# paullric/tempestmodel

Measured on AMD Instinct MI355X. Metric: element-DOF-updates/s (JW baroclinic wave ne30 np4 L30, ARS343 IMEX), higher is better.
Workload: dtype f64

## Files before the change

include/tempest_mi355x.h:

```cpp
#ifndef TEMPEST_MI355X_H
#define TEMPEST_MI355X_H

#ifdef __cplusplus
extern "C" {
#endif

#define TMX_ABI_VERSION 5

#define TMX_OK                 0
#define TMX_ERR_INVALID       -1
#define TMX_ERR_UNSUPPORTED   -2
#define TMX_ERR_DEVICE        -3
#define TMX_ERR_SINGULAR      -4
#define TMX_ERR_COMM          -5

typedef struct tmx_engine tmx_engine;

enum {
	TMX_OP_INTERP_NODE_TO_REDGE = 0,
	TMX_OP_INTERP_REDGE_TO_NODE,
	TMX_OP_DIFF_NODE_TO_NODE,
	TMX_OP_DIFF_NODE_TO_REDGE,
	TMX_OP_DIFF_REDGE_TO_NODE,
	TMX_OP_DIFF_REDGE_TO_REDGE,
// ... 181 lines not shown
	TMX_INFO_COLUMN_KERNEL,
	TMX_INFO_COLUMN_VARIANT
};
long long tmx_info(tmx_engine * e, int what);

int tmx_set_option(tmx_engine * e, const char * name, double value);
int tmx_get_option(tmx_engine * e, const char * name, double * value);
typedef void (*tmx_dgbsv_fn)(const int * n, const int * kl, const int * ku, const int * nrhs, double * ab, const int * ldab, int * ipiv,
	double * b, const int * ldb, int * info);
int tmx_lu_flavour_from_dgbsv(tmx_engine * e, tmx_dgbsv_fn dgbsv);
int tmx_options_report(tmx_engine * e, char * buf, int cap);
int tmx_options_from_environment(tmx_engine * e);

int tmx_plan_get(tmx_engine * e, int what, int * out, int cap);
int tmx_plan_get_matrices(tmx_engine * e, double * out, int cap);
int tmx_debug_unique_tables(tmx_engine * e, int tile_shape, int what, int * out, int cap);
int tmx_debug_program_unique(int scheme, int first_step, int last_step);
int tmx_debug_program_mixed(int scheme, int first_step, int last_step, int instance);
int tmx_debug_program_rayleigh(int scheme, int first_step, int last_step);
int tmx_debug_program_prefix(int scheme, int first_step, int last_step, int * pairs, int * terms, int cap);
int tmx_debug_h_timing(tmx_engine * e, unsigned long long * out);
int tmx_debug_h_walk_timing(tmx_engine * e, unsigned long long * out);

int tmx_debug_dss_loopback(tmx_engine ** engines, int n, int instance);
int tmx_debug_loopback_group(tmx_engine ** engines, int n);
int tmx_debug_comm_selftest(tmx_engine * e);

int tmx_debug_pivot_stats(tmx_engine * e, int enable, unsigned long long out[2]);

int tmx_debug_program_copies(int scheme, int mode, int steps, int share, int * copies, int * shared);
int tmx_debug_dcmip_node_coefficients(int panel, double alpha, double beta, double * out);
int tmx_debug_dcmip_tsurf(double lat, double * out);

enum {
	TMX_K_H_EXPLICIT = 0, TMX_K_V_EXPLICIT, TMX_K_VI_ASSEMBLE, TMX_K_VI_SOLVE, TMX_K_DSS,
	TMX_K_HYPERVIS, TMX_K_LINCOMB, TMX_K_EXCHANGE, TMX_K_COUNT
};
int tmx_profile_enable(tmx_engine * e, int on);
int tmx_profile_get(tmx_engine * e, int kernel, double * total_ms, long long * launches);
int tmx_profile_reset(tmx_engine * e);

#ifdef __cplusplus
}
#endif
#endif
```

tempestmodel_amd/csrc/tmx_host.hip:

```cpp
#include "tmx_hostshared.h"


static thread_local std::string g_err;

void tmx_set_error(const char * fmt, ...) {
	char buf[1024];
	va_list ap;
	va_start(ap, fmt);
	vsnprintf(buf, sizeof(buf), fmt, ap);
	va_end(ap);
	g_err = buf;
}

extern "C" const char * tmx_last_error(void) { return g_err.c_str(); }




NcclApi g_nccl;

int load_rccl() {
	if (g_nccl.Send) return TMX_OK;
	void * h = dlopen(nullptr, RTLD_NOW | RTLD_GLOBAL);
	if (!h || !dlsym(h, "ncclSend")) {
// ... 884 lines not shown
			int n = 0;
			if (e->comm && g_nccl.CommCount && g_nccl.CommCount(e->comm, &n) == 0) return n;
			return 0;
		}
		case TMX_INFO_SEND_COLUMNS: return e->nsend;
		case TMX_INFO_HALO_TRANSPORT: return (e->cfg.n_ranks == 1) ? 0 : (e->lb ? 3 : (e->p2p ? 2 : (e->comm ? 1 : 0)));
	}
	return -1;
}

extern "C" int tmx_debug_h_timing(tmx_engine * e, unsigned long long * out) {
	int r; if ((r = check_ready(e))) return r;
	HIPCHK(hipStreamSynchronize(e->stream));
	tmxk_h_timing_read(out);
	return TMX_OK;
}
extern "C" int tmx_debug_h_walk_timing(tmx_engine * e, unsigned long long * out) {
	int r; if ((r = check_ready(e))) return r;
	HIPCHK(hipStreamSynchronize(e->stream));
	tmxk_h_walk_timing_read(out);
	return TMX_OK;
}

extern "C" int tmx_debug_pivot_stats(tmx_engine * e, int enable, unsigned long long out[2]) {
	int r; if ((r = check_ready(e))) return r;
	HIPCHK(hipStreamSynchronize(e->stream));
	if (out) {
		out[0] = out[1] = 0;
		if (e->d_pivot_stats) HIPCHK(hipMemcpy(out, e->d_pivot_stats, 2 * sizeof(unsigned long long), hipMemcpyDeviceToHost));
	}
#ifdef TMX_PAIR_TIMING
	const size_t stat_words = 2 + 8 * 4096;
	if (e->d_pivot_stats && !enable) {
		std::vector<unsigned long long> rec(stat_words);
		HIPCHK(hipMemcpy(rec.data(), e->d_pivot_stats, stat_words * sizeof(unsigned long long), hipMemcpyDeviceToHost));
		for (size_t w = 0; w < 4096; w++) {
			const unsigned long long * q = &rec[2 + 8 * w];
			if (q[0]) fprintf(stderr, "pairtiming wave %zu role %llu hw_id %llx xcc %llu work %llu wait %llu forward %llu back %llu\n", w, q[0] - 1, q[1], q[2], q[3], q[4], q[5], q[6]);
		}
		if (e->vi_split_back) {
			const int n = TMX_FTOT * (e->L + 1);
			for (int g : { 0, 100, 400 }) {
				std::vector<int> m(n);
				HIPCHK(hipMemcpy(m.data(), (const int *)e->d_rhs + (size_t)g * n, n * sizeof(int), hipMemcpyDeviceToHost));
				fprintf(stderr, "umask group %d:", g);
				for (int j = 0; j < n; j++) fprintf(stderr, " %x", m[j] >> 4);
// ... 34 lines not shown
```

tempestmodel_amd/csrc/tmx_internal.h:

```cpp
#pragma once
#include <hip/hip_runtime.h>
#include <string>
#include <vector>
#include "../../include/tempest_mi355x.h"

#define TMX_NP 4
#define TMX_NQ 16
#define TMX_TILE 64
#define TMX_FLAG_SINGULAR 1
#define TMX_FLAG_COMM 2
#define TMX_FTOT 3
#define TMX_BW 9

#define TMX_SLAB_U(L,k) (k)
#define TMX_SLAB_V(L,k) ((L) + (k))
#define TMX_SLAB_T(L,k) (2 * (L) + (k))
#define TMX_SLAB_R(L,k) (3 * (L) + (k))
#define TMX_SLAB_W(L,k) (4 * (L) + (k))
#define TMX_SLAB_Q(L,c,k) (5 * (L) + 1 + (c) * (L) + (k))

enum { G2_J2D = 0, G2_F, G2_C2A0, G2_C2A1, G2_C2B1, G2_JN, G2_JE, G2_DRX, G2_ZS,
	G2_LAT, G2_PS,
	G2_SINLAT, G2_COSLAT,
	G2_MP, G2_MA, G2_MB, G2_MC, G2_DAZ, G2_DBZ, G2_IDX, G2_IDX2,
// ... 58 lines not shown
	int b_ngroups = 0, b_ngroups_local = 0, nblocks = 0, nb_early = 0, nb_late = 0;
	int * d_b_sdst = nullptr, * d_b_sred = nullptr, * d_blk_info = nullptr, * d_b_gsrc = nullptr, * d_b_gdst = nullptr, * d_b_gn = nullptr, * d_b_gx = nullptr, * d_b_gtype = nullptr;
	int * d_blks_early = nullptr, * d_blks_late = nullptr;
	bool vite_ok = true;
	bool slots_by_blocks = false;
	int block_option = -1;
	size_t ustride = 0;
	double * d_ustate = nullptr, * d_part = nullptr, * d_g2d_t = nullptr, * d_g2d_u = nullptr;
	int * d_t_ucol = nullptr, * d_t_sdst = nullptr, * d_t_sred = nullptr;
	int * d_t_tinfo = nullptr;
	int * d_t_dcol = nullptr;
	int * d_ucol_of_dcol = nullptr;
	int * d_u_rep = nullptr;
	int * d_slot_ucol = nullptr;
	int * d_gsrc = nullptr, * d_gdst = nullptr, * d_gn = nullptr, * d_gx = nullptr, * d_gtype = nullptr;
	int * d_send_slots = nullptr;
	int * d_quads_early = nullptr, * d_quads_late = nullptr; int n_early = 0, n_late = 0; bool split = false;
	int * d_check = nullptr;
	std::vector<char> form;
	std::vector<int> uslot; int uspare = 0;
	int uprefix = 0, prefix_option = 1;
	long long prefix_for = -1;
	long long prefix_stages = 0;
	int n_uform = 0;
	long long conversions = 0;
	int backoff = 0, skip_steps = 0;
	unsigned dlive = 0u;
	int mixed_option = 1;
	long long mixed_steps = 0;
	bool physics_dirty = true, physics_ok = false;
	double * d_surf_u = nullptr;
};

struct PlanHost {
	std::vector<int> grp_cols, grp_n, grp_x, grp_type;
	std::vector<double> xmat;
	std::vector<int> send_nodes;
	std::vector<int> recv_nodes;
	std::vector<int> send_cols;
	std::vector<int> ucol, udep;
	std::vector<int> colref;
	std::vector<int> hvblocks;
	std::vector<int> quads_early, quads_late;
	std::vector<int> send_base, send_stride, ghost_base, ghost_stride;
};

// ... 155 lines not shown
#define TMX_EXP 1
#else
#define TMX_EXP 0
#endif
static inline bool tmxu_blocks_on(const tmx_engine * e, int which = 0) {
	if (!TMX_EXP || !e->u.built) return false;
	const int o = e->u.block_option;
	if (o == 2) return which != 2;
	if (o == 3) return which != 1;
	return o == 1 || (o < 0 && e->u.tile_shape == 4);
}

struct EmitTerms { double * xp; double coef[12]; int first; };
void tmxk_h_explicit(tmx_engine * e, const KParams & p, const double * xin, const double * xbase, double * xup, double dt, int fuse_v,
	int nterms = 0, const double * const * src = nullptr, const double * coef = nullptr, int premul = 0,
	const double * xin_uv = nullptr, const double * xbase_uv = nullptr, const double * const * src_uv = nullptr, const EmitTerms * emit = nullptr,
	unsigned dmask = 0u);
bool tmxk_h_walk_ok(const tmx_engine * e, const KParams & p, int fuse_v, int nterms, bool emit);
void tmxk_h_walk_prepare(tmx_engine * e, const KParams & p);
int tmxk_h_walk_segments(const tmx_engine * e, const KParams & p, int ntiles, int nterms, int waves_per_simd = 0);
void tmxk_h_walk(tmx_engine * e, const KParams & p, const double * xin, const double * xbase, double * xup, double dt, int fuse_v,
	int nterms, const double * const * src, const double * coef, int premul, const double * xin_uv, const double * xbase_uv, const double * const * src_uv, unsigned dmask,
	const EmitTerms * emit = nullptr);
bool tmxk_h_walk_fuses_udiff(const tmx_engine * e, const KParams & p, int fuse_v, int nterms);
bool tmxk_hv_walk_ok(const tmx_engine * e, const KParams & p);
void tmxk_hv_walk(tmx_engine * e, const KParams & p, const double * xsrc, const double * xbase, double * xout, double dt, double nu_s, double nu_d, double nu_v, int scale);
void tmxk_h_walk_timing_read(unsigned long long * out);
void tmxk_h_timing_read(unsigned long long * out);
void tmxk_sw_explicit(tmx_engine * e, const KParams & p, const double * xin, const double * xbase, double * xup, double dt);
void tmxk_v_explicit(tmx_engine * e, const KParams & p, const double * xin, double * xup, double dt, bool with_udiff_uv = false);
void tmxk_vi_assemble(tmx_engine * e, const KParams & p, const double * xin, double dt);
void tmxk_vi_solve(tmx_engine * e, const KParams & p, const double * xin, double * xup);
void tmxk_vi_fused(tmx_engine * e, const KParams & p, const double * xin, double * xup, double dt);
void tmxk_vi_terms_explicit(tmx_engine * e, const KParams & p, const double * xin, double * xup, double dt, bool with_uv = false);
void tmxk_dss(tmx_engine * e, const KParams & p, double * x, int g0, int g1);
void tmxk_hypervis(tmx_engine * e, const KParams & p, const double * xsrc, const double * xbase, double * xout,
	double dt, double nu_s, double nu_d, double nu_v, int scale_locally, bool pull_dss = false);
void tmxk_lincomb(tmx_engine * e, size_t n, double * dst, int nterms, const double * const * src, const double * coef, int dst_is_term0);
void tmxk_pack(tmx_engine * e, const KParams & p, const double * x);
void tmxk_pack_p2p(tmx_engine * e, const KParams & p, const double * x, int buf);
void tmxk_p2p_signal_wait(tmx_engine * e, hipStream_t s, int buf, unsigned long long seq);
void tmxk_rayleigh(tmx_engine * e, const KParams & p, double * x, double dt, const double * xs = nullptr, size_t NSS = 0, const int * ucd = nullptr);
void tmxk_held_suarez(tmx_engine * e, const KParams & p, double * x, const double * surf, double dt, const double * xs = nullptr, size_t NSS = 0, const int * ucd = nullptr);
void tmxk_kessler(tmx_engine * e, const KParams & p, double * x, double dt);
enum { DC_RA0 = 0, DC_RA1, DC_RB0, DC_RB1, DC_RCOS, DC_ADIV, DC_AA0, DC_AA1, DC_AB0, DC_AB1, DC_TSURF1, TMX_DC_NCOEF };
#define TMX_DC_NW 20
// ... 25 lines not shown
```

tempestmodel_amd/csrc/tmx_k_hwalk.hip:

```cpp
#include "tmx_device.h"

#ifdef TMX_H_TIMING
#define HW_WAVES 32768
__device__ unsigned long long g_hw_rec[8][HW_WAVES][8];
#define HW_DECL long long hw_ = __builtin_readcyclecounter(); long long hws_[7] = { 0, 0, 0, 0, 0, 0, 0 }
#define HW_MARK(i) do { const long long t1_ = __builtin_readcyclecounter(); hws_[i] += t1_ - hw_; hw_ = t1_; } while (0)
#define HW_END(NT_) do { if (threadIdx.x == 0) { const unsigned w_ = blockIdx.x % HW_WAVES; \
	for (int q_ = 0; q_ < 7; q_++) g_hw_rec[(NT_) & 7][w_][q_] = (unsigned long long)hws_[q_]; g_hw_rec[(NT_) & 7][w_][7] = 1ull; } } while (0)
void tmxk_h_walk_timing_read(unsigned long long * out) {
	static std::vector<unsigned long long> h((size_t)8 * HW_WAVES * 8);
	hipMemcpyFromSymbol(h.data(), HIP_SYMBOL(g_hw_rec), h.size() * sizeof(unsigned long long));
	for (int i = 0; i < 128; i++) out[i] = 0;
	for (int nt = 0; nt < 8; nt++) for (int w = 0; w < HW_WAVES; w++) if (h[((size_t)nt * HW_WAVES + w) * 8 + 7])
		for (int q = 0; q < 8; q++) out[nt * 8 + q] += h[((size_t)nt * HW_WAVES + w) * 8 + q];
	std::fill(h.begin(), h.end(), 0ull);
	hipMemcpyToSymbol(HIP_SYMBOL(g_hw_rec), h.data(), h.size() * sizeof(unsigned long long));
}
#else
#define HW_DECL
#define HW_MARK(i)
#define HW_END(NT_)
void tmxk_h_walk_timing_read(unsigned long long * out) { for (int i = 0; i < 128; i++) out[i] = 0; }
#endif

template <bool DM>
__device__ __forceinline__ double term_load(const double * src, unsigned dmask, int m, int slab, size_t SS, size_t NS, unsigned cb, unsigned gb) {
	const bool d = DM && ((dmask >> m) & 1u);
	return ldu_term(src + (size_t)slab * (d ? NS : SS), d ? gb : cb);
}

template <int NT, bool PM, bool DM>
__device__ __forceinline__ void terms_load(const double * const (&src)[12], unsigned dmask, int slab, size_t SS, size_t NS, unsigned cb, unsigned gb, double (&x)[NT > 0 ? NT : 1]) {
	if (NT == 0) { x[0] = term_load<DM>(src[0], dmask, 0, slab, SS, NS, cb, gb); return; }
#pragma unroll
	for (int m = 0; m < NT; m++) x[m] = (m > 0 || PM) ? term_load<DM>(src[m], dmask, m, slab, SS, NS, cb, gb) : 0.0;
}

typedef const double __attribute__((address_space(4))) * tmx_cdp;
#define OPK(op, k, off) opsc[(((op) * (L + 1)) + (k)) * TMX_OPW + ((off) + 2)]

#ifndef TMX_HW_WAVES_PER_EU
#define TMX_HW_WAVES_PER_EU 2
#endif

struct UdiffArgs { const double * xref; double ks, kv; const double * xrefd; double cfv; int udv; };
#define TMX_REFD_HU(L, k) (k)
#define TMX_REFD_HV(L, k) ((L) + (k))
#define TMX_REFD_DU(L, k) (2 * (L) + (k))
#define TMX_REFD_DV(L, k) (3 * (L) + (k))

__global__ __launch_bounds__(64) void k_ref_diffusion_terms(KParams p, const double * __restrict__ xref, double * __restrict__ xrefd, double kv)
{
	__shared__ double s[4][64];
	__shared__ double sD[16], sS[16];
	const int lane = threadIdx.x;
	if (lane < 16) { sD[lane] = p.dx[lane]; sS[lane] = p.stiff[lane]; }
	const int L = p.L, k = blockIdx.y;
	const size_t NS = (size_t)p.NS;
// ... 24 lines not shown
#pragma unroll
	for (int t = 0; t < 4; t++) {
		const int la = eb + 4 * t + j, lb = eb + 4 * i + t;
		const double Sa = sS[i * 4 + t], Sb = sS[j * 4 + t];
		dadr -= Sa * s[0][la]; dbdr -= Sb * s[0][lb];
		dacr -= Sa * s[1][la]; dbcr -= Sb * s[1][lb];
	}
	dadr *= ida; dbdr *= idb; dacr *= ida; dbcr *= idb;
	const double upar = kv * dadr - kv * j2d * (c2a1 * dacr + c2b1 * dbcr);
	const double upbr = kv * dbdr + kv * j2d * (c2a0 * dacr + c2a1 * dbcr);
	double ddr[2] = { 0.0, 0.0 };
#pragma unroll
	for (int off = -2; off <= 2; off++) {
		const int l = k + off;
		if (l < 0 || l >= L) continue;
		const double c = p.ops[((TMX_OP_DIFFDIFF_NODE_TO_NODE * (L + 1)) + k) * TMX_OPW + (off + 2)];
		ddr[0] += c * xref[TMX_SLAB_U(L, l) * NS + col];
		ddr[1] += c * xref[TMX_SLAB_V(L, l) * NS + col];
	}
	if (!here) return;
	xrefd[TMX_REFD_HU(L, k) * NS + col] = upar; xrefd[TMX_REFD_HV(L, k) * NS + col] = upbr;
	xrefd[TMX_REFD_DU(L, k) * NS + col] = ddr[0]; xrefd[TMX_REFD_DV(L, k) * NS + col] = ddr[1];
}
template <int NT, bool PM, bool DM, bool BLK = false, bool EM = false, bool UQ = true, bool FV = true, bool UD = false>
__global__ __launch_bounds__(BLK ? 256 : 64, TMX_HW_WAVES_PER_EU) void k_h_walk(KParams p, const double * __restrict__ xin, LinTerms xbase, double * xup, double dt, UvTerms uvt, int nseg, EmitTerms em,
	UdiffArgs ud)
{
	constexpr int RL = TMX_UQ_ROWLEN(true);
	constexpr int NW = BLK ? 4 : 1;
	__shared__ double sw[NW][9][RL];
	__shared__ double xs[BLK ? 2 : 1][BLK ? 6 : 1][BLK ? 256 : 1];
	__shared__ double sD[16], sS[16];
	__shared__ double rmtab[TMX_RMTAB_DOUBLES];
	const int wv = BLK ? WAVE_UNIFORM(threadIdx.y) : 0;
	double (*s)[RL] = sw[wv];
	const int lane = tile_lane<true>();
	const int lp = lds_pos<true>(lane);
	HW_DECL;
	constexpr int NTL = BLK ? 1 : 4;
	double tlog[NTL]; unsigned long long texp[NTL];
	const int tidw = wv * 64 + (int)threadIdx.x;
#pragma unroll
	for (int t = 0; t < NTL; t++) { tlog[t] = tmx_rm_log_tab[t * 64 + tidw]; texp[t] = tmx_rm_exp_tab[t * 64 + tidw]; }
	const int L = p.L;
	const size_t NS = (size_t)p.NS, SS = UQ ? (size_t)p.NSS : NS, NSD = (size_t)p.NSD;
	int tix, seg;
	if (!wg_tile<UQ>(p, nseg, tix, seg)) return;
// ... 72 lines not shown
		ve += OPK(TMX_OP_INTERP_NODE_TO_REDGE, k0, -1) * vM; ve += OPK(TMX_OP_INTERP_NODE_TO_REDGE, k0, 0) * v0;
		double e0, e1, e2, ea, eb_;
		met_eval(mc, etac[L + k0], e0, e1, e2, ea, eb_);
		xlo = e0 * ue + e1 * ve + e2 * w0;
		wave_sync();
	}
	double uh0 = 0.0, vh0 = 0.0;
	HW_MARK(0);

	constexpr int NX = NT > 0 ? NT : 1;
	for (int kl = k0; kl < k1; kl++) {
		const int k = WAVE_UNIFORM(kl);
		asm volatile("" : "+v"(cb), "+v"(gd), "+v"(cx));
		double uN = uP, vN = vP, wN = 0.0, tN = 0.0, rN = 0.0;
		if (k + 1 < k1 || (FV && UD && k + 2 < L)) {
			const int kpp = (k + 2 < L) ? k + 2 : L - 1;
			uN = ldu(xuv + TMX_SLAB_U(L, kpp) * SX, cx); vN = ldu(xuv + TMX_SLAB_V(L, kpp) * SX, cx);
		}
		if (k + 1 < k1) {
			wN = ldu(xin + TMX_SLAB_W(L, k + 2) * SX, cx);
			tN = ldu(xin + TMX_SLAB_T(L, k + 1) * SX, cx); rN = ldu(xin + TMX_SLAB_R(L, k + 1) * SX, cx);
		}
		double xU[NX], xV[NX], xT[NX], xR[NX], xW[NX];
		terms_load<NT, PM, DM>(uvt.src, dmask, TMX_SLAB_U(L, k), SS, NSD, cb, gd, xU);
		terms_load<NT, PM, DM>(uvt.src, dmask, TMX_SLAB_V(L, k), SS, NSD, cb, gd, xV);
		terms_load<NT, PM, DM>(xbase.src, dmask, TMX_SLAB_T(L, k), SS, NSD, cb, gd, xT);
		terms_load<NT, PM, DM>(xbase.src, dmask, TMX_SLAB_R(L, k), SS, NSD, cb, gd, xR);
		terms_load<NT, PM, DM>(xbase.src, dmask, TMX_SLAB_W(L, (k > 0) ? k : 1), SS, NSD, cb, gd, xW);
		double rfT = 0.0, rfW = 0.0, hdU = 0.0, hdV = 0.0, ddU = 0.0, ddV = 0.0;
		if (UD) {
			rfT = ldu(ud.xref + TMX_SLAB_T(L, k) * NS, cb); rfW = ldu(ud.xref + TMX_SLAB_W(L, k) * NS, cb);
			hdU = ldu(ud.xrefd + TMX_REFD_HU(L, k) * NS, cb); hdV = ldu(ud.xrefd + TMX_REFD_HV(L, k) * NS, cb);
			if (FV && ud.udv) { ddU = ldu(ud.xrefd + TMX_REFD_DU(L, k) * NS, cb); ddV = ldu(ud.xrefd + TMX_REFD_DV(L, k) * NS, cb); }
		}
		__builtin_amdgcn_sched_barrier(0);
		HW_MARK(1);

		double ca2, cb2, cx2, dra, drb;
		met_eval(mc, etac[k], ca2, cb2, cx2, dra, drb);
		double ux = 0.0; ux += OPK(TMX_OP_INTERP_REDGE_TO_NODE, k, 0) * w0; ux += OPK(TMX_OP_INTERP_REDGE_TO_NODE, k, 1) * w1;
		const double conUa = c2a0 * u0 + c2a1 * v0 + ca2 * ux;
		const double conUb = c2a1 * u0 + c2b1 * v0 + cb2 * ux;
		const double conUx = ca2 * u0 + cb2 * v0 + cx2 * ux;
		const double dm = OPK(TMX_OP_DIFF_NODE_TO_NODE, k, -1), d0 = OPK(TMX_OP_DIFF_NODE_TO_NODE, k, 0), dp = OPK(TMX_OP_DIFF_NODE_TO_NODE, k, 1);
		double dxua = 0.0; dxua += dm * uM; dxua += d0 * u0; dxua += dp * uP;
		double dxub = 0.0; dxub += dm * vM; dxub += d0 * v0; dxub += dp * vP;
		double xhi = 0.0;
		if (FV && k + 1 <= L - 1) {
			double ue = 0.0, ve = 0.0;
			ue += OPK(TMX_OP_INTERP_NODE_TO_REDGE, k + 1, -1) * u0; ue += OPK(TMX_OP_INTERP_NODE_TO_REDGE, k + 1, 0) * uP;
			ve += OPK(TMX_OP_INTERP_NODE_TO_REDGE, k + 1, -1) * v0; ve += OPK(TMX_OP_INTERP_NODE_TO_REDGE, k + 1, 0) * vP;
// ... 184 lines not shown
			if (k == 1) {
				double ub0 = 0.0, vb0 = 0.0;
				ub0 += OPK(TMX_OP_INTERP_NODE_TO_REDGE, 0, 0) * uh0; ub0 += OPK(TMX_OP_INTERP_NODE_TO_REDGE, 0, 1) * uh;
				vb0 += OPK(TMX_OP_INTERP_NODE_TO_REDGE, 0, 0) * vh0; vb0 += OPK(TMX_OP_INTERP_NODE_TO_REDGE, 0, 1) * vh;
				double e0, e1, e2, ea, eb_;
				met_eval(mc, etac[L], e0, e1, e2, ea, eb_);
				double wb = -(e0 * ub0 + e1 * vb0) / e2;
				if (UD) wb = wb - xW0;
				if (here) stu(xup + TMX_SLAB_W(L, 0) * NS, cb, wb);
			}
		} else if constexpr (BLK) {
			double extra = 0.0; int xslab = TMX_SLAB_W(L, 0); unsigned vmask = (k > 0) ? 31u : 15u;
			if (k == 0) { uh0 = uh; vh0 = vh; }
			if (k == 1) {
				double ub0 = 0.0, vb0 = 0.0;
				ub0 += OPK(TMX_OP_INTERP_NODE_TO_REDGE, 0, 0) * uh0; ub0 += OPK(TMX_OP_INTERP_NODE_TO_REDGE, 0, 1) * uh;
				vb0 += OPK(TMX_OP_INTERP_NODE_TO_REDGE, 0, 0) * vh0; vb0 += OPK(TMX_OP_INTERP_NODE_TO_REDGE, 0, 1) * vh;
				double e0, e1, e2, ea, eb_;
				met_eval(mc, etac[L], e0, e1, e2, ea, eb_);
				extra = -(e0 * ub0 + e1 * vb0) / e2; vmask |= 32u;
			}
			if (k == L - 1) {
				double xWl[NX];
				terms_load<NT, PM, DM>(xbase.src, dmask, TMX_SLAB_W(L, L), SS, NSD, cb, gd, xWl);
				extra = lin_reduce<NT, PM>(xbase, xWl); xslab = TMX_SLAB_W(L, L); vmask |= 32u;
				if (EM) stu(em.xp + TMX_SLAB_W(L, L) * SS, cb, emit_value<NT>(em, xWl));
			}
			const double v[6] = { outU, outV, outR, outT, outW, extra };
			const int slab[6] = { TMX_SLAB_U(L, k), TMX_SLAB_V(L, k), TMX_SLAB_R(L, k), TMX_SLAB_T(L, k), TMX_SLAB_W(L, k), xslab };
			block_seam_store<6>(p, xs[k & 1], pos, sdst, sred, v, xup, slab, vmask);
		} else {
			{
				const double v[5] = { outU, outV, outR, outT, outW };
				const int slab[5] = { TMX_SLAB_U(L, k), TMX_SLAB_V(L, k), TMX_SLAB_R(L, k), TMX_SLAB_T(L, k), TMX_SLAB_W(L, k) };
				seam_store<5, RL>(p, &s[0], lane, sdst, sred, v, xup, slab, (k > 0) ? 5 : 4);
			}
			if (k == 0) { uh0 = uh; vh0 = vh; }
			if (k == 1) {
				wave_sync();
				double ub0 = 0.0, vb0 = 0.0;
				ub0 += OPK(TMX_OP_INTERP_NODE_TO_REDGE, 0, 0) * uh0; ub0 += OPK(TMX_OP_INTERP_NODE_TO_REDGE, 0, 1) * uh;
				vb0 += OPK(TMX_OP_INTERP_NODE_TO_REDGE, 0, 0) * vh0; vb0 += OPK(TMX_OP_INTERP_NODE_TO_REDGE, 0, 1) * vh;
				double e0, e1, e2, ea, eb_;
				met_eval(mc, etac[L], e0, e1, e2, ea, eb_);
				const double v1[1] = { -(e0 * ub0 + e1 * vb0) / e2 };
				const int slab1[1] = { TMX_SLAB_W(L, 0) };
				seam_store<1, RL>(p, &s[0], lane, sdst, sred, v1, xup, slab1, 1);
			}
		}
		wave_sync();
		HW_MARK(6);
		if (FV && UD) { uMM = uM; vMM = vM; }
		uM = u0; u0 = uP; uP = uN; vM = v0; v0 = vP; vP = vN;
		w0 = w1; w1 = wN; t0 = tN; r0 = rN;
		ucz_prev = uczx; xlo = xhi;
	}
	if (!BLK && k1 == L) {
		double xW[NX];
		terms_load<NT, PM, DM>(xbase.src, dmask, TMX_SLAB_W(L, L), SS, NSD, cb, gd, xW);
		const double v1[1] = { lin_reduce<NT, PM>(xbase, xW) };
		if constexpr (!UQ) {
			double wl = v1[0];
			if constexpr (UD) {
				const double psiW = w0 - ldu(ud.xref + TMX_SLAB_W(L, L) * NS, cb);
				wave_sync();
				s[1][lp] = psiW;
				wave_sync();
				double daW = 0, dbW = 0;
#pragma unroll
				for (int t = 0; t < 4; t++) { daW += s[1][eb + 4 * t + j] * sD[t * 4 + i]; dbW += s[1][eb + 4 * i + t] * sD[t * 4 + j]; }
				daW *= ida; dbW *= idb;
				wave_sync();
				s[2][lp] = je * (c2a0 * daW + c2a1 * dbW); s[3][lp] = je * (c2a1 * daW + c2b1 * dbW);
				wave_sync();
				double uaW = 0, ubW = 0;
#pragma unroll
				for (int t = 0; t < 4; t++) { uaW += s[2][eb + 4 * t + j] * sS[i * 4 + t]; ubW += s[3][eb + 4 * i + t] * sS[j * 4 + t]; }
				uaW *= ida; ubW *= idb;
				wl = wl - dt * (1.0 / je) * ud.kv * (uaW + ubW);
			}
			if (here) stu(xup + TMX_SLAB_W(L, L) * NS, cb, wl);
			HW_MARK(6); HW_END(NT); return;
// ... 33 lines not shown
}

bool tmxk_h_walk_fuses_udiff(const tmx_engine * e, const KParams & p, int fuse_v, int nterms) {
	return e->udiff && !p.t_ucol && (fuse_v ? e->opt_h_walk_udiff >= 2 : e->opt_h_walk_udiff != 0) && tmxk_h_walk_ok(e, p, fuse_v, nterms, false);
}

static const double * ref_diffusion_terms(tmx_engine * e, const KParams & p) {
	if (!e->d_refd) {
		const size_t rb = (size_t)4 * p.L * p.NS * sizeof(double);
		if (hipMalloc((void **)&e->d_refd, rb) != hipSuccess) { e->d_refd = nullptr; return nullptr; }
		hipMemsetAsync(e->d_refd, 0, rb, e->stream);
		e->hbm_bytes += rb; e->refd_valid = false;
	}
	if (!e->refd_valid) {
		KParams q = p; q.quads = nullptr;
		hipLaunchKernelGGL(k_ref_diffusion_terms, dim3(p.NS / 64, p.L), dim3(64), 0, e->stream, q, (const double *)e->d_ref, e->d_refd, e->cfg.uniform_diffusion_vector);
		e->refd_valid = true;
	}
	return e->d_refd;
}

void tmxk_h_walk_prepare(tmx_engine * e, const KParams & p) {
	if (e->udiff && !e->refd_valid && e->d_ref && tmxk_h_walk_fuses_udiff(e, p, 0, 0)) (void)ref_diffusion_terms(e, p);
}

void tmxk_h_walk(tmx_engine * e, const KParams & p, const double * xin, const double * xbase_ptr, double * xup, double dt, int fuse_v,
	int nterms, const double * const * src, const double * coef, int premul, const double * xin_uv, const double * xbase_uv, const double * const * src_uv, unsigned dmask,
	const EmitTerms * emit) {
	LinTerms xbase;
	UvTerms uvt;
	xbase.n = nterms; xbase.premul = premul; xbase.dmask = dmask;
	xbase.src[0] = xbase_ptr; xbase.coef[0] = 0.0;
	uvt.xin = xin_uv ? xin_uv : xin; uvt.src[0] = xbase_uv ? xbase_uv : xbase_ptr;
	for (int m = 0; m < nterms; m++) { xbase.src[m] = src[m]; xbase.coef[m] = coef[m]; uvt.src[m] = src_uv ? src_uv[m] : src[m]; }
	for (int m = (nterms > 0 ? nterms : 1); m < 12; m++) { xbase.src[m] = xbase.src[0]; xbase.coef[m] = 0.0; uvt.src[m] = uvt.src[0]; }
	const int ntile = p.quads ? e->launch_tiles : p.NS / 64;
	const int nseg = tmxk_h_walk_segments(e, p, ntile, nterms, ((!p.t_ucol && tmxk_h_walk_fuses_udiff(e, p, fuse_v, nterms)) || (nterms == 2 && premul)) ? 2 : 0);
	KParams q = p; q.u_ntiles = ntile;
	if (!p.t_ucol) {
		EmitTerms em1; em1.xp = nullptr; em1.first = -1; for (int m = 0; m < 12; m++) em1.coef[m] = 0.0;
		const dim3 grd(ntile, nseg), blk(64);
		const bool udf = tmxk_h_walk_fuses_udiff(e, p, fuse_v, nterms);
		const UdiffArgs ud0 = { nullptr, 0.0, 0.0, nullptr, 0.0, 0 }, ud1 = { (const double *)e->d_ref, e->cfg.uniform_diffusion_scalar, e->cfg.uniform_diffusion_vector,
			udf ? ref_diffusion_terms(e, p) : nullptr, e->cfg.uniform_diffusion_vector / (e->cfg.ztop * e->cfg.ztop), (e->fully_explicit && !e->opt_udv_separate) ? 1 : 0 };
#define LAUNCH_D2(NT_, PM_) do { \
			if (fuse_v && udf) hipLaunchKernelGGL((k_h_walk<NT_, PM_, false, false, false, false, true, true>), grd, blk, 0, e->stream, q, xin, xbase, xup, dt, uvt, nseg, em1, ud1); \
			else if (fuse_v) hipLaunchKernelGGL((k_h_walk<NT_, PM_, false, false, false, false, true>), grd, blk, 0, e->stream, q, xin, xbase, xup, dt, uvt, nseg, em1, ud0); \
			else if (udf) hipLaunchKernelGGL((k_h_walk<NT_, PM_, false, false, false, false, false, true>), grd, blk, 0, e->stream, q, xin, xbase, xup, dt, uvt, nseg, em1, ud1); \
			else hipLaunchKernelGGL((k_h_walk<NT_, PM_, false, false, false, false, false>), grd, blk, 0, e->stream, q, xin, xbase, xup, dt, uvt, nseg, em1, ud0); } while (0)
#define LAUNCH_D(NT_) do { if (NT_ == 0 || premul) LAUNCH_D2(NT_, true); else LAUNCH_D2(NT_, false); } while (0)
		switch (nterms) {
			case 0: LAUNCH_D(0); break;
			case 2: LAUNCH_D(2); break;
			case 3: LAUNCH_D(3); break;
			case 4: LAUNCH_D(4); break;
			case 5: LAUNCH_D(5); break;
			case 6: LAUNCH_D(6); break;
			case 7: LAUNCH_D(7); break;
			default: LAUNCH_D(8); break;
		}
#undef LAUNCH_D
#undef LAUNCH_D2
		return;
	}
	const bool blocks = tmxu_blocks_on(e, 1) && p.L >= 3;
	const int nblk = p.bquads ? e->launch_blocks : e->u.nblocks;
	if (blocks) q.u_ntiles = nblk;
	e->u.slots_by_blocks = blocks;
	const dim3 blk(64, blocks ? 4 : 1), grd = wg_grid(true, q, blocks ? nblk : ntile, nseg);
	EmitTerms em0; em0.xp = nullptr; em0.first = -1; for (int m = 0; m < 12; m++) em0.coef[m] = 0.0;
	const UdiffArgs udn = { nullptr, 0.0, 0.0, nullptr, 0.0, 0 };
	const bool emit_ok = emit && emit->xp && !premul && !dmask && !blocks && nterms >= 3 && nterms <= 8;
	const EmitTerms em = emit_ok ? *emit : em0;
#define LAUNCH_W3(NT_, PM_, DM_) do { \
		if (emit_ok && NT_ >= 3 && !PM_ && !DM_) hipLaunchKernelGGL((k_h_walk<(NT_ >= 3 ? NT_ : 3), false, false, false, true>), grd, blk, 0, e->stream, q, xin, xbase, xup, dt, uvt, nseg, em, udn); \
		else if (TMX_EXP && blocks) hipLaunchKernelGGL((k_h_walk<NT_, PM_, DM_, TMX_EXP != 0>), grd, blk, 0, e->stream, q, xin, xbase, xup, dt, uvt, nseg, em0, udn); \
		else hipLaunchKernelGGL((k_h_walk<NT_, PM_, DM_, false>), grd, blk, 0, e->stream, q, xin, xbase, xup, dt, uvt, nseg, em0, udn); } while (0)
#define LAUNCH_W2(NT_, PM_) do { if (dmask) LAUNCH_W3(NT_, PM_, true); else LAUNCH_W3(NT_, PM_, false); } while (0)
#define LAUNCH_W(NT_) do { if (NT_ == 0 || premul) LAUNCH_W2(NT_, true); else LAUNCH_W2(NT_, false); } while (0)
	switch (nterms) {
		case 0: LAUNCH_W(0); break;
		case 2: LAUNCH_W(2); break;
		case 3: LAUNCH_W(3); break;
		case 4: LAUNCH_W(4); break;
		case 5: LAUNCH_W(5); break;
		case 6: LAUNCH_W(6); break;
		case 7: LAUNCH_W(7); break;
		default: LAUNCH_W(8); break;
	}
#undef LAUNCH_W3
#undef LAUNCH_W
#undef LAUNCH_W2
}

template <bool HB>
__global__ __launch_bounds__(64, 4) void k_hv_walk(KParams p, const double * __restrict__ xsrc, const double * __restrict__ xbase, double * __restrict__ xout,
// ... 129 lines not shown
```

tempestmodel_amd/engine.py:

```python
import ctypes as C
import os
import numpy as np

_HERE = os.path.dirname(os.path.abspath(__file__))
LIB_PATH = os.environ.get("TMX_LIBRARY") or os.path.join(_HERE, "libtempest_mi355x.so")

TMX_ABI_VERSION = 5
OP_NAMES = ["interp_node_to_redge", "interp_redge_to_node", "diff_node_to_node", "diff_node_to_redge",
            "diff_redge_to_node", "diff_redge_to_redge", "diffdiff_node_to_node", "diffdiff_redge_to_redge",
            "penalty_left", "penalty_right"]
GEOM_FIELDS = ["jacobian2d", "contra_metric_2d_a", "contra_metric_2d_b", "jacobian", "jacobian_redge",
               "contra_metric_a", "contra_metric_b", "contra_metric_xi",
               "contra_metric_a_redge", "contra_metric_b_redge", "contra_metric_xi_redge",
               "deriv_r_node", "deriv_r_redge", "coriolis_f", "topography", "element_area_node"]
KERNEL_NAMES = ["h_explicit", "v_explicit", "vi_assemble", "vi_solve", "dss", "hypervis", "lincomb", "exchange"]

PD = C.POINTER(C.c_double)
PI = C.POINTER(C.c_int)


class TempestError(RuntimeError):

    def __init__(self, code, msg):
        super().__init__("tempest_mi355x error %d: %s" % (code, msg))
# ... 62 lines not shown
    lib.tmx_profile_get.argtypes = [C.c_void_p, C.c_int, PD, C.POINTER(C.c_longlong)]
    lib.tmx_upload_state.argtypes = [C.c_void_p, C.c_int, C.c_int, PD, PD]
    lib.tmx_download_state.argtypes = [C.c_void_p, C.c_int, C.c_int, PD, PD]
    lib.tmx_set_patch_metric_factors.argtypes = [C.c_void_p, C.c_int, PD, PD, PD, C.c_double, PD, PD]
    lib.tmx_set_patch_rayleigh.argtypes = [C.c_void_p, C.c_int, PD, PD, PD, PD]
    lib.tmx_set_patch_reference_state.argtypes = [C.c_void_p, C.c_int, PD, PD, PD]
    lib.tmx_v_filter_negative_tracers.argtypes = [C.c_void_p, C.c_int]
    lib.tmx_interp_create.argtypes = [C.c_void_p, C.POINTER(TmxInterpPoints), C.POINTER(C.c_void_p)]
    lib.tmx_interp_destroy.argtypes = [C.c_void_p]
    lib.tmx_interp_destroy.restype = None
    lib.tmx_interp_state.argtypes = [C.c_void_p, C.c_void_p, C.c_int, C.c_int, C.c_int, C.c_int, C.c_double, PD]
    lib.tmx_interp_tracers.argtypes = [C.c_void_p, C.c_void_p, C.c_int, PD]
    lib.tmx_h_substep_after_subcycle.argtypes = [C.c_void_p, C.c_int, C.c_int, C.c_int, C.c_double, C.c_int, C.POINTER(C.c_int)]
    lib.tmx_h_substep_after_subcycle_count.argtypes = [C.c_void_p]
    lib.tmx_set_patch_physics_inputs.argtypes = [C.c_void_p, C.c_int, PD, PD]
    lib.tmx_physics_held_suarez.argtypes = [C.c_void_p, C.c_int, C.c_double]
    lib.tmx_set_patch_level_heights.argtypes = [C.c_void_p, C.c_int, PD]
    lib.tmx_active_state_bytes.argtypes = [C.c_void_p, C.c_int]
    lib.tmx_active_state_bytes.restype = C.c_longlong
    lib.tmx_pack_active_state.argtypes = [C.c_void_p, C.c_int, C.c_int, C.c_void_p, C.c_size_t]
    lib.tmx_unpack_active_state.argtypes = [C.c_void_p, C.c_int, C.c_int, C.c_void_p, C.c_size_t]
    lib.tmx_set_strang_off_centering.argtypes = [C.c_void_p, C.c_double]
    lib.tmx_debug_pivot_stats.argtypes = [C.c_void_p, C.c_int, C.POINTER(C.c_ulonglong)]
    lib.tmx_set_patch_element_spacing.argtypes = [C.c_void_p, C.c_int, C.c_double, C.c_double]
    lib.tmx_physics_kessler.argtypes = [C.c_void_p, C.c_int, C.c_double]
    lib.tmx_download_precipitation.argtypes = [C.c_void_p, C.c_int, PD, C.c_int]
    lib.tmx_set_patch_dcmip_inputs.argtypes = [C.c_void_p, C.c_int, PD, PD, PD, PD, C.c_double]
    lib.tmx_physics_dcmip2016.argtypes = [C.c_void_p, C.c_int, C.c_double, C.c_int, C.c_int, C.c_int]
    lib.tmx_debug_dcmip_node_coefficients.argtypes = [C.c_int, C.c_double, C.c_double, PD]
    lib.tmx_debug_dcmip_tsurf.argtypes = [C.c_double, PD]
    lib.tmx_upload_tracers.argtypes = [C.c_void_p, C.c_int, C.c_int, PD]
    lib.tmx_download_tracers.argtypes = [C.c_void_p, C.c_int, C.c_int, PD]
    lib.tmx_comm_init.argtypes = [C.c_void_p, C.c_char_p]
    lib.tmx_halo_p2p_blob_bytes.argtypes = [C.c_void_p]
    lib.tmx_halo_p2p_export.argtypes = [C.c_void_p, C.c_char_p]
    lib.tmx_halo_p2p_connect.argtypes = [C.c_void_p, C.c_char_p]
    lib.tmx_halo_p2p_enable.argtypes = [C.c_void_p, C.c_int]
    lib.tmx_halo_p2p_reset.argtypes = [C.c_void_p]
    lib.tmx_comm_unique_id.argtypes = [C.c_char_p]
    lib.tmx_set_option.argtypes = [C.c_void_p, C.c_char_p, C.c_double]
    lib.tmx_get_option.argtypes = [C.c_void_p, C.c_char_p, PD]
    lib.tmx_options_from_environment.argtypes = [C.c_void_p]
    lib.tmx_options_report.argtypes = [C.c_void_p, C.c_char_p, C.c_int]
    _libs[path] = lib
    return lib

# ... 167 lines not shown
            out[p] = (n, e)
        return out

    def set_physics_inputs(self, surface_pressure=None):
        for p in self.local_patches:
            P = self.grid.patches[p]
            la = np.ascontiguousarray(P.lat, dtype=np.float64)
            sp = None if surface_pressure is None else np.ascontiguousarray(surface_pressure[p], dtype=np.float64)
            self._chk(self.lib.tmx_set_patch_physics_inputs(self.h, p, _pd(la), None if sp is None else _pd(sp)))

    def held_suarez(self, instance, dt):
        self._chk(self.lib.tmx_physics_held_suarez(self.h, instance, dt))

    def set_level_heights(self, z_levels=None):
        for p in self.local_patches:
            z = np.ascontiguousarray(self.grid.patches[p].geom["z_levels"] if z_levels is None else z_levels[p], dtype=np.float64)
            self._chk(self.lib.tmx_set_patch_level_heights(self.h, p, _pd(z)))

    def pivot_stats(self, enable):
        out = (C.c_ulonglong * 2)()
        self._chk(self.lib.tmx_debug_pivot_stats(self.h, 1 if enable else 0, out))
        return int(out[0]), int(out[1])

    def kessler(self, instance, dt):
        self._chk(self.lib.tmx_physics_kessler(self.h, instance, dt))

    def set_dcmip_inputs(self, latitude=None, a_nodes=None, b_nodes=None, z_interfaces=None, earth_radius=None):
        a = self.grid.phys.earth_radius if earth_radius is None else earth_radius
        for p in self.local_patches:
            P = self.grid.patches[p]
            la = np.ascontiguousarray(P.lat if latitude is None else latitude[p], dtype=np.float64)
            an = np.ascontiguousarray(P.a_nodes if a_nodes is None else a_nodes[p], dtype=np.float64)
            bn = np.ascontiguousarray(P.b_nodes if b_nodes is None else b_nodes[p], dtype=np.float64)
            zi = np.ascontiguousarray(P.geom["z_interfaces"] if z_interfaces is None else z_interfaces[p], dtype=np.float64)
            self._chk(self.lib.tmx_set_patch_dcmip_inputs(self.h, p, _pd(la), _pd(an), _pd(bn), _pd(zi), float(a)))

    def dcmip2016(self, instance, dt, test, pbl_type, prec_type):
        self._chk(self.lib.tmx_physics_dcmip2016(self.h, instance, dt, test, pbl_type, prec_type))

    def download_precipitation(self, reset=False):
        out = {}
        for p in self.local_patches:
            P = self.grid.patches[p]
            a = np.zeros((P.na, P.nb))
            self._chk(self.lib.tmx_download_precipitation(self.h, p, _pd(a), 1 if reset else 0))
            out[p] = a
# ... 296 lines not shown
```

Before: 11.52 billion.

## Reuse window values and duplicate term loads in horizontal walk kernel

Adds a compile-time reuse descriptor to the horizontal walk kernel. When a linear-combination source pointer equals the input state, or repeats an earlier term, the kernel reuses the already-loaded window value or the earlier term instead of issuing another global load. The host checks pointer identities on each launch and picks one of a fixed set of specialised kernel instantiations, falling back to the generic path otherwise. This cuts redundant memory traffic in IMEX stage combinations, at the cost of more template instantiations and host-side dispatch logic, plus debug counters.

```diff
diff --git a/include/tempest_mi355x.h b/include/tempest_mi355x.h
--- a/include/tempest_mi355x.h
+++ b/include/tempest_mi355x.h
@@ -227,6 +227,10 @@
 int tmx_debug_h_timing(tmx_engine * e, unsigned long long * out);
 int tmx_debug_h_walk_timing(tmx_engine * e, unsigned long long * out);
 
+int tmx_debug_walk_reuse_plan(int nterms, int premul, unsigned dmask, int blocks, int unique, int emit, long long xin, long long xin_uv,
+	const long long * src, const long long * src_uv, unsigned long long * desc);
+int tmx_debug_walk_reuse_counts(tmx_engine * e, long long out[2]);
+
 int tmx_debug_dss_loopback(tmx_engine ** engines, int n, int instance);
 int tmx_debug_loopback_group(tmx_engine ** engines, int n);
 int tmx_debug_comm_selftest(tmx_engine * e);
diff --git a/tempestmodel_amd/csrc/tmx_host.hip b/tempestmodel_amd/csrc/tmx_host.hip
--- a/tempestmodel_amd/csrc/tmx_host.hip
+++ b/tempestmodel_amd/csrc/tmx_host.hip
@@ -930,6 +930,20 @@
 	return TMX_OK;
 }
 
+extern "C" int tmx_debug_walk_reuse_plan(int nterms, int premul, unsigned dmask, int blocks, int unique, int emit, long long xin, long long xin_uv,
+	const long long * src, const long long * src_uv, unsigned long long * desc) {
+	REQUIRE(src && src_uv && desc && (nterms == 0 || (nterms >= 2 && nterms <= 8)), TMX_ERR_INVALID, "tmx_debug_walk_reuse_plan: bad argument");
+	unsigned long long a[12], b[12];
+	for (int m = 0; m < 12; m++) { const int q = m < (nterms ? nterms : 1) ? m : 0; a[m] = (unsigned long long)src[q]; b[m] = (unsigned long long)src_uv[q]; }
+	*desc = tmxk_h_walk_reuse(nterms, premul, dmask, blocks != 0, unique != 0, (unsigned long long)xin, (unsigned long long)xin_uv, a, b);
+	return tmxk_h_walk_reuse_form(nterms, premul, emit != 0, *desc) >= 0 ? 1 : 0;
+}
+extern "C" int tmx_debug_walk_reuse_counts(tmx_engine * e, long long out[2]) {
+	REQUIRE(e && out, TMX_ERR_INVALID, "tmx_debug_walk_reuse_counts: null argument");
+	out[0] = e->u.walk_reuse; out[1] = e->u.walk_plain;
+	return TMX_OK;
+}
+
 extern "C" int tmx_debug_pivot_stats(tmx_engine * e, int enable, unsigned long long out[2]) {
 	int r; if ((r = check_ready(e))) return r;
 	HIPCHK(hipStreamSynchronize(e->stream));
diff --git a/tempestmodel_amd/csrc/tmx_internal.h b/tempestmodel_amd/csrc/tmx_internal.h
--- a/tempestmodel_amd/csrc/tmx_internal.h
+++ b/tempestmodel_amd/csrc/tmx_internal.h
@@ -104,6 +104,7 @@
 	int uprefix = 0, prefix_option = 1;
 	long long prefix_for = -1;
 	long long prefix_stages = 0;
+	long long walk_reuse = 0, walk_plain = 0;
 	int n_uform = 0;
 	long long conversions = 0;
 	int backoff = 0, skip_steps = 0;
@@ -305,6 +306,16 @@
 void tmxk_h_walk(tmx_engine * e, const KParams & p, const double * xin, const double * xbase, double * xup, double dt, int fuse_v,
 	int nterms, const double * const * src, const double * coef, int premul, const double * xin_uv, const double * xbase_uv, const double * const * src_uv, unsigned dmask,
 	const EmitTerms * emit = nullptr);
+typedef unsigned long long tmx_reuse_t;
+enum { TMX_RU_LOAD = 0, TMX_RU_WIN = 1 };
+#define TMX_RU_TERM(j) (2 + (j))
+#define TMX_RU(m, uv, rest) ((tmx_reuse_t)((uv) | (rest) << 4) << (8 * (m)))
+#ifndef TMX_H_WALK_REUSE
+#define TMX_H_WALK_REUSE 1
+#endif
+tmx_reuse_t tmxk_h_walk_reuse(int nterms, int premul, unsigned dmask, bool blocks, bool unique, unsigned long long xin, unsigned long long xin_uv,
+	const unsigned long long * src, const unsigned long long * src_uv);
+int tmxk_h_walk_reuse_form(int nterms, int premul, bool emit, tmx_reuse_t ru);
 bool tmxk_h_walk_fuses_udiff(const tmx_engine * e, const KParams & p, int fuse_v, int nterms);
 bool tmxk_hv_walk_ok(const tmx_engine * e, const KParams & p);
 void tmxk_hv_walk(tmx_engine * e, const KParams & p, const double * xsrc, const double * xbase, double * xout, double dt, double nu_s, double nu_d, double nu_v, int scale);
diff --git a/tempestmodel_amd/csrc/tmx_k_hwalk.hip b/tempestmodel_amd/csrc/tmx_k_hwalk.hip
--- a/tempestmodel_amd/csrc/tmx_k_hwalk.hip
+++ b/tempestmodel_amd/csrc/tmx_k_hwalk.hip
@@ -29,11 +29,16 @@
 	return ldu_term(src + (size_t)slab * (d ? NS : SS), d ? gb : cb);
 }
 
-template <int NT, bool PM, bool DM>
-__device__ __forceinline__ void terms_load(const double * const (&src)[12], unsigned dmask, int slab, size_t SS, size_t NS, unsigned cb, unsigned gb, double (&x)[NT > 0 ? NT : 1]) {
-	if (NT == 0) { x[0] = term_load<DM>(src[0], dmask, 0, slab, SS, NS, cb, gb); return; }
-#pragma unroll
-	for (int m = 0; m < NT; m++) x[m] = (m > 0 || PM) ? term_load<DM>(src[m], dmask, m, slab, SS, NS, cb, gb) : 0.0;
+template <int NT, bool PM, bool DM, tmx_reuse_t RU = 0, bool UV = false>
+__device__ __forceinline__ void terms_load(const double * const (&src)[12], unsigned dmask, int slab, size_t SS, size_t NS, unsigned cb, unsigned gb, double win, double (&x)[NT > 0 ? NT : 1]) {
+#pragma unroll
+	for (int m = 0; m < (NT > 0 ? NT : 1); m++) {
+		const int st = (int)(RU >> (8 * m + (UV ? 0 : 4)) & 15u);
+		if (NT > 0 && m == 0 && !PM) x[m] = 0.0;
+		else if (st == TMX_RU_LOAD) x[m] = term_load<DM>(src[m], dmask, m, slab, SS, NS, cb, gb);
+		else if (st == TMX_RU_WIN) x[m] = win;
+		else x[m] = x[st - 2 < m ? st - 2 : 0];
+	}
 }
 
 typedef const double __attribute__((address_space(4))) * tmx_cdp;
@@ -104,7 +109,7 @@
 	xrefd[TMX_REFD_HU(L, k) * NS + col] = upar; xrefd[TMX_REFD_HV(L, k) * NS + col] = upbr;
 	xrefd[TMX_REFD_DU(L, k) * NS + col] = ddr[0]; xrefd[TMX_REFD_DV(L, k) * NS + col] = ddr[1];
 }
-template <int NT, bool PM, bool DM, bool BLK = false, bool EM = false, bool UQ = true, bool FV = true, bool UD = false>
+template <int NT, bool PM, bool DM, bool BLK = false, bool EM = false, bool UQ = true, bool FV = true, bool UD = false, tmx_reuse_t RU = 0>
 __global__ __launch_bounds__(BLK ? 256 : 64, TMX_HW_WAVES_PER_EU) void k_h_walk(KParams p, const double * __restrict__ xin, LinTerms xbase, double * xup, double dt, UvTerms uvt, int nseg, EmitTerms em,
 	UdiffArgs ud)
 {
@@ -223,11 +228,11 @@
 			tN = ldu(xin + TMX_SLAB_T(L, k + 1) * SX, cx); rN = ldu(xin + TMX_SLAB_R(L, k + 1) * SX, cx);
 		}
 		double xU[NX], xV[NX], xT[NX], xR[NX], xW[NX];
-		terms_load<NT, PM, DM>(uvt.src, dmask, TMX_SLAB_U(L, k), SS, NSD, cb, gd, xU);
-		terms_load<NT, PM, DM>(uvt.src, dmask, TMX_SLAB_V(L, k), SS, NSD, cb, gd, xV);
-		terms_load<NT, PM, DM>(xbase.src, dmask, TMX_SLAB_T(L, k), SS, NSD, cb, gd, xT);
-		terms_load<NT, PM, DM>(xbase.src, dmask, TMX_SLAB_R(L, k), SS, NSD, cb, gd, xR);
-		terms_load<NT, PM, DM>(xbase.src, dmask, TMX_SLAB_W(L, (k > 0) ? k : 1), SS, NSD, cb, gd, xW);
+		terms_load<NT, PM, DM, RU, true>(uvt.src, dmask, TMX_SLAB_U(L, k), SS, NSD, cb, gd, u0, xU);
+		terms_load<NT, PM, DM, RU, true>(uvt.src, dmask, TMX_SLAB_V(L, k), SS, NSD, cb, gd, v0, xV);
+		terms_load<NT, PM, DM, RU>(xbase.src, dmask, TMX_SLAB_T(L, k), SS, NSD, cb, gd, t0, xT);
+		terms_load<NT, PM, DM, RU>(xbase.src, dmask, TMX_SLAB_R(L, k), SS, NSD, cb, gd, r0, xR);
+		terms_load<NT, PM, DM, RU>(xbase.src, dmask, TMX_SLAB_W(L, (k > 0) ? k : 1), SS, NSD, cb, gd, (k > 0) ? w0 : w1, xW);
 		double rfT = 0.0, rfW = 0.0, hdU = 0.0, hdV = 0.0, ddU = 0.0, ddV = 0.0;
 		if (UD) {
 			rfT = ldu(ud.xref + TMX_SLAB_T(L, k) * NS, cb); rfW = ldu(ud.xref + TMX_SLAB_W(L, k) * NS, cb);
@@ -458,7 +463,7 @@
 			}
 			if (k == L - 1) {
 				double xWl[NX];
-				terms_load<NT, PM, DM>(xbase.src, dmask, TMX_SLAB_W(L, L), SS, NSD, cb, gd, xWl);
+				terms_load<NT, PM, DM>(xbase.src, dmask, TMX_SLAB_W(L, L), SS, NSD, cb, gd, 0.0, xWl);
 				extra = lin_reduce<NT, PM>(xbase, xWl); xslab = TMX_SLAB_W(L, L); vmask |= 32u;
 				if (EM) stu(em.xp + TMX_SLAB_W(L, L) * SS, cb, emit_value<NT>(em, xWl));
 			}
@@ -493,7 +498,7 @@
 	}
 	if (!BLK && k1 == L) {
 		double xW[NX];
-		terms_load<NT, PM, DM>(xbase.src, dmask, TMX_SLAB_W(L, L), SS, NSD, cb, gd, xW);
+		terms_load<NT, PM, DM, RU>(xbase.src, dmask, TMX_SLAB_W(L, L), SS, NSD, cb, gd, w0, xW);
 		const double v1[1] = { lin_reduce<NT, PM>(xbase, xW) };
 		if constexpr (!UQ) {
 			double wl = v1[0];
@@ -573,6 +578,48 @@
 
 void tmxk_h_walk_prepare(tmx_engine * e, const KParams & p) {
 	if (e->udiff && !e->refd_valid && e->d_ref && tmxk_h_walk_fuses_udiff(e, p, 0, 0)) (void)ref_diffusion_terms(e, p);
+}
+
+tmx_reuse_t tmxk_h_walk_reuse(int nterms, int premul, unsigned dmask, bool blocks, bool unique, unsigned long long xin, unsigned long long xin_uv,
+	const unsigned long long * src, const unsigned long long * src_uv) {
+	if (!TMX_H_WALK_REUSE || dmask || blocks || !unique || nterms < 0 || nterms == 1 || nterms > 8) return 0;
+	tmx_reuse_t ru = 0;
+	for (int m = 0; m < (nterms ? nterms : 1); m++) {
+		if (nterms && m == 0 && !premul) continue;
+		int uv = TMX_RU_LOAD;
+		if (src_uv[m] == xin_uv) uv = TMX_RU_WIN;
+		else for (int j = m - 1; j >= (premul ? 0 : 1); j--) if (src_uv[j] == src_uv[m]) uv = TMX_RU_TERM(j);
+		ru |= TMX_RU(m, uv, src[m] == xin ? TMX_RU_WIN : TMX_RU_LOAD);
+	}
+	return ru;
+}
+
+#define RU_L TMX_RU_LOAD
+#define RU_W TMX_RU_WIN
+#define RU_T(j) TMX_RU_TERM(j)
+#define TMX_WALK_REUSE_FORMS(X) \
+	 \
+	X(0, true, false, TMX_RU(0, RU_W, RU_W)) \
+	 \
+	X(4, false, false, TMX_RU(2, RU_W, RU_L) | TMX_RU(3, RU_W, RU_W)) \
+	 \
+	X(6, false, true, TMX_RU(3, RU_T(2), RU_L) | TMX_RU(4, RU_W, RU_L) | TMX_RU(5, RU_W, RU_W)) \
+	 \
+	X(3, true, false, TMX_RU(1, RU_W, RU_L) | TMX_RU(2, RU_W, RU_W)) \
+	 \
+	X(4, false, false, TMX_RU(3, RU_W, RU_W)) \
+	 \
+	X(7, false, false, TMX_RU(4, RU_W, RU_L) | TMX_RU(5, RU_W, RU_W)) \
+	 \
+	X(7, false, false, TMX_RU(5, RU_W, RU_W))
+
+int tmxk_h_walk_reuse_form(int nterms, int premul, bool emit, tmx_reuse_t ru) {
+	const bool pm = nterms == 0 || premul != 0;
+	int row = 0;
+#define X(NT_, PM_, EM_, RU_) if (ru && nterms == NT_ && pm == PM_ && emit == EM_ && ru == (RU_)) return row; row++;
+	TMX_WALK_REUSE_FORMS(X)
+#undef X
+	return -1;
 }
 
 void tmxk_h_walk(tmx_engine * e, const KParams & p, const double * xin, const double * xbase_ptr, double * xup, double dt, int fuse_v,
@@ -589,6 +636,7 @@
 	const int nseg = tmxk_h_walk_segments(e, p, ntile, nterms, ((!p.t_ucol && tmxk_h_walk_fuses_udiff(e, p, fuse_v, nterms)) || (nterms == 2 && premul)) ? 2 : 0);
 	KParams q = p; q.u_ntiles = ntile;
 	if (!p.t_ucol) {
+		e->u.walk_plain++;
 		EmitTerms em1; em1.xp = nullptr; em1.first = -1; for (int m = 0; m < 12; m++) em1.coef[m] = 0.0;
 		const dim3 grd(ntile, nseg), blk(64);
 		const bool udf = tmxk_h_walk_fuses_udiff(e, p, fuse_v, nterms);
@@ -623,6 +671,16 @@
 	const UdiffArgs udn = { nullptr, 0.0, 0.0, nullptr, 0.0, 0 };
 	const bool emit_ok = emit && emit->xp && !premul && !dmask && !blocks && nterms >= 3 && nterms <= 8;
 	const EmitTerms em = emit_ok ? *emit : em0;
+	unsigned long long ids[12], ids_uv[12];
+	for (int m = 0; m < 12; m++) { ids[m] = (unsigned long long)xbase.src[m]; ids_uv[m] = (unsigned long long)uvt.src[m]; }
+	const tmx_reuse_t ru = tmxk_h_walk_reuse(nterms, premul, dmask, blocks, true, (unsigned long long)xin, (unsigned long long)uvt.xin, ids, ids_uv);
+	const int form = tmxk_h_walk_reuse_form(nterms, premul, emit_ok, ru);
+	int row = 0;
+#define X(NT_, PM_, EM_, RU_) if (form == row++) { e->u.walk_reuse++; \
+		hipLaunchKernelGGL((k_h_walk<NT_, PM_, false, false, EM_, true, true, false, (RU_)>), grd, blk, 0, e->stream, q, xin, xbase, xup, dt, uvt, nseg, em, udn); return; }
+	TMX_WALK_REUSE_FORMS(X)
+#undef X
+	e->u.walk_plain++;
 #define LAUNCH_W3(NT_, PM_, DM_) do { \
 		if (emit_ok && NT_ >= 3 && !PM_ && !DM_) hipLaunchKernelGGL((k_h_walk<(NT_ >= 3 ? NT_ : 3), false, false, false, true>), grd, blk, 0, e->stream, q, xin, xbase, xup, dt, uvt, nseg, em, udn); \
 		else if (TMX_EXP && blocks) hipLaunchKernelGGL((k_h_walk<NT_, PM_, DM_, TMX_EXP != 0>), grd, blk, 0, e->stream, q, xin, xbase, xup, dt, uvt, nseg, em0, udn); \
diff --git a/tempestmodel_amd/engine.py b/tempestmodel_amd/engine.py
--- a/tempestmodel_amd/engine.py
+++ b/tempestmodel_amd/engine.py
@@ -108,6 +108,10 @@
     lib.tmx_unpack_active_state.argtypes = [C.c_void_p, C.c_int, C.c_int, C.c_void_p, C.c_size_t]
     lib.tmx_set_strang_off_centering.argtypes = [C.c_void_p, C.c_double]
     lib.tmx_debug_pivot_stats.argtypes = [C.c_void_p, C.c_int, C.POINTER(C.c_ulonglong)]
+    if hasattr(lib, "tmx_debug_walk_reuse_counts"):
+        lib.tmx_debug_walk_reuse_counts.argtypes = [C.c_void_p, C.POINTER(C.c_longlong)]
+        lib.tmx_debug_walk_reuse_plan.argtypes = [C.c_int, C.c_int, C.c_uint, C.c_int, C.c_int, C.c_int, C.c_longlong, C.c_longlong,
+                                                  C.POINTER(C.c_longlong), C.POINTER(C.c_longlong), C.POINTER(C.c_ulonglong)]
     lib.tmx_set_patch_element_spacing.argtypes = [C.c_void_p, C.c_int, C.c_double, C.c_double]
     lib.tmx_physics_kessler.argtypes = [C.c_void_p, C.c_int, C.c_double]
     lib.tmx_download_precipitation.argtypes = [C.c_void_p, C.c_int, PD, C.c_int]
@@ -321,6 +325,11 @@
         self._chk(self.lib.tmx_debug_pivot_stats(self.h, 1 if enable else 0, out))
         return int(out[0]), int(out[1])
 
+    def walk_reuse_counts(self):
+        out = (C.c_longlong * 2)()
+        self._chk(self.lib.tmx_debug_walk_reuse_counts(self.h, out))
+        return int(out[0]), int(out[1])
+
     def kessler(self, instance, dt):
         self._chk(self.lib.tmx_physics_kessler(self.h, instance, dt))
 
```

After: 11.85 billion, median of 6. +2.8%, better.
